# AmadeusChan/test-nccl-p2p

Hardware: AMD Instinct MI355X
Metric: pairwise P2P GB/s matrix (min/mean) + p50 latency at 1/2/4/8 MI355X (higher is better)
Workload: dtype uint8

## Files before the change

csrc/pymodule.cpp:

```cpp
#include <hip/hip_runtime.h>

#include <pybind11/pybind11.h>
#include <pybind11/stl.h>

#include <chrono>
#include <cstdlib>
#include <memory>
#include <string>
#include <thread>
#include <tuple>
#include <vector>

#include "app.hpp"
#include "bootstrap.hpp"
#include "common.hpp"
#include "kernels.hpp"
#include "provenance.hpp"
#include "report.hpp"
#include "runner.hpp"
#include "routing.hpp"
#include "schedule.hpp"
#include "transport.hpp"
#include "units.hpp"

// ... 136 lines not shown
    if (device) return ring_latency_to_json(run_device_ring_latency(*t_, *boot_, bytes, laps, warmup));
    Buffers bufs(*t_, std::max<size_t>(bytes, 16), 1);
    return ring_latency_to_json(run_ring_latency(*t_, *boot_, bytes, laps, warmup, bufs));
  }

  void set_timeout(double seconds) {
    t_->set_timeout(seconds);
    boot_->set_timeout(seconds);
  }

  bool set_chunk_cap(size_t bytes) { return t_->set_chunk_cap(bytes); }
  size_t max_chunk(int peer) const { return t_->max_chunk(peer); }
  bool refine_op_limits() { return t_->refine_op_limits(*boot_); }

  std::string link_reports() {
    const auto all = boot_->allgather_string(t_->link_report());
    std::string o = "[";
    for (size_t r = 0; r < all.size(); ++r) o += (r ? "," : "") + (all[r].empty() ? std::string("null") : all[r]);
    return o + "]";
  }

  std::string provenance(int device) { return provenance_json(*boot_, device); }

 private:
  std::unique_ptr<Bootstrap> boot_;
  std::unique_ptr<Transport> t_;
  std::string transport_kind_;
  uint64_t salt_ = 1000;
};

class PyStepDriver {
 public:
  PyStepDriver(std::shared_ptr<Session> s, const std::string& mode, const std::string& dir, size_t bytes, int msgs,
               bool verify, bool batch, bool graph, int depth, size_t recv_budget, uint64_t salt)
      : session_(std::move(s)),
        d_(std::make_unique<StepDriver>(session_->t(), session_->boot(),
                                        make_schedule(parse_mode(mode), parse_direction(dir), session_->world()),
                                        bytes, msgs, verify, salt, StepOptions{batch, graph, depth, recv_budget})) {}
  ~PyStepDriver() {
    teardown_outside_gil([this] {
      if (!session_->t().drain_quietly()) {
        (void)d_.release();
        return;
      }
      d_.reset();
    });
  }
  StepDriver& d() { return *d_; }

 private:
  std::shared_ptr<Session> session_;
  std::unique_ptr<StepDriver> d_;
};

hipStream_t as_stream(uintptr_t s) { return reinterpret_cast<hipStream_t>(s); }

struct KernelScratch {
  dev::VerifyAccum* d = nullptr;
  dev::VerifyAccum* h = nullptr;
  int device = -1;
};
KernelScratch& scratch() {
  static KernelScratch s;
  int dv = 0;
  if (hipGetDevice(&dv) != hipSuccess) P2P_FATAL("no HIP device");
  if (s.device != dv) {
    if (s.d) (void)hipFree(s.d);
    if (s.h) (void)hipHostFree(s.h);
    if (hipMalloc(&s.d, dev::verify_accum_bytes()) != hipSuccess) P2P_FATAL("hipMalloc failed");
    if (hipHostMalloc(&s.h, sizeof(dev::VerifyAccum), hipHostMallocDefault) != hipSuccess) P2P_FATAL("hipHostMalloc failed");
    s.device = dv;
// ... 228 lines not shown
      .def("device_latency", &Session::device_latency, py::arg("bytes") = 8, py::arg("iters") = 1000,
           py::arg("warmup") = 100, py::call_guard<NativeCall, py::gil_scoped_release>())
      .def("latency", &Session::latency, py::arg("bytes") = 8, py::arg("iters") = 1000, py::arg("warmup") = 100,
           py::arg("preposted") = 0, py::call_guard<NativeCall, py::gil_scoped_release>(),
           "Ping-pong matrix (collective).  preposted=B: exchanges posted B at a time behind a stream gate and "
           "released together (GPU-timeline latency; host-posted where the transport has no gate).")
      .def("fuzz", &Session::fuzz, py::arg("rounds") = 20, py::arg("seed") = 1, py::arg("max_bytes") = size_t{4} << 20,
           py::call_guard<NativeCall, py::gil_scoped_release>(),
           "Random groups of verified messages through the transport (collective); returns mismatching words.")
      .def("ring_latency", &Session::ring_latency, py::arg("bytes") = 8, py::arg("laps") = 200, py::arg("warmup") = 20,
           py::arg("device") = false, py::call_guard<NativeCall, py::gil_scoped_release>(),
           "Dependent ring token chain 0 -> 1 -> ... -> 0 (collective); JSON with per-hop and per-lap times.")
      .def("set_timeout", &Session::set_timeout, py::arg("seconds"),
           "Bounds every later wait of the session (transport sync / rendezvous, bootstrap receives).")
      .def("set_chunk_cap", &Session::set_chunk_cap, py::arg("bytes"),
           "Caps the ops messages to every peer are posted as at `bytes` (0: lifts the cap, back to the limits the "
           "transport derived per peer); False where nothing is split. Call it on every rank with the same value.")
      .def("max_chunk", &Session::max_chunk, py::arg("peer"), "Largest op a message to `peer` is posted as (0: unsplit).")
      .def("refine_op_limits", &Session::refine_op_limits, py::call_guard<NativeCall, py::gil_scoped_release>(),
           "Collective: op limits from the connections made so far (RCCL: its connection lines).")
      .def("link_reports", &Session::link_reports, py::call_guard<NativeCall, py::gil_scoped_release>(),
           "Collective: what the data plane set up towards each peer, per rank (RCCL: p2p channels from its INFO log, "
           "each peer's transport, the op limit in use); JSON list.")
      .def("provenance", &Session::provenance, py::arg("device") = -1, py::call_guard<NativeCall, py::gil_scoped_release>(),
           "Collective: runtime, RCCL library, knobs, every rank's GPU and the links between them (JSON).")
      .def("_post_unmatched_recv", &Session::post_unmatched_recv, py::arg("bytes"), py::arg("peer"),
           py::call_guard<NativeCall, py::gil_scoped_release>(),
           "Test hook: a receive no send matches, left pending; the session's teardown must still end.")
      .def("_unmatched_recv", &Session::unmatched_recv, py::arg("bytes") = size_t{1} << 20,
           py::call_guard<NativeCall, py::gil_scoped_release>(), "Test hook: a receive no send matches; returns the watchdog's error.");

  py::class_<PyStepDriver>(m, "StepDriver")
      .def(py::init<std::shared_ptr<Session>, const std::string&, const std::string&, size_t, int, bool, bool, bool, int,
                    size_t, uint64_t>(),
           py::arg("session"), py::arg("mode") = "tournament", py::arg("dir") = "bi", py::arg("bytes") = 32u << 20,
           py::arg("msgs") = 8, py::arg("verify") = false, py::arg("batch") = false, py::arg("graph") = false,
           py::arg("depth") = 1, py::arg("recv_budget") = size_t{0}, py::arg("salt") = uint64_t{0},
           py::call_guard<NativeCall, py::gil_scoped_release>())
      .def("poison", [](PyStepDriver& s) { s.d().poison(); }, py::call_guard<NativeCall, py::gil_scoped_release>(),
           "Collective: zero every receive slot (after the warmup, before the timed steps) and arm the skip faults.")
      .def("clear", [](PyStepDriver& s) { s.d().clear(); }, py::call_guard<NativeCall, py::gil_scoped_release>(),
           "Collective: zero every receive slot once every rank has drained (no fault armed).")
      .def("recapture", [](PyStepDriver& s) { s.d().recapture(); }, py::call_guard<NativeCall, py::gil_scoped_release>(),
           "Collective: record the step graphs again after the op sizes changed (no-op without graphs).")
      .def_property_readonly("recaptures", [](PyStepDriver& s) { return s.d().recaptures(); })
      .def_property_readonly("limit_changes", [](PyStepDriver& s) { return s.d().limit_changes(); })
      .def_property_readonly("graphs", [](PyStepDriver& s) { return s.d().graphs(); })
      .def("verify_steps", [](PyStepDriver& s, long first, long count) {
            StepVerifyReport r;
            {
              NativeCall in_engine;
              py::gil_scoped_release nogil;
              r = s.d().verify_steps(first, count);
            }
            py::dict d;
            d["mismatches"] = r.mismatches;
            d["verified_msgs"] = r.verified_msgs;
            d["timed_msgs"] = r.timed_msgs;
            d["slots"] = r.slots;
            return d;
          }, py::arg("first"), py::arg("count"),
           "Collective: checks every receive slot steps [first, first+count) wrote (all ranks' totals).")
      .def("flows_per_step", [](PyStepDriver& s, long k) { return s.d().flows_per_step(k); })
      .def_property_readonly("depth", [](PyStepDriver& s) { return s.d().depth(); })
      .def_property_readonly("msgs", [](PyStepDriver& s) { return s.d().msgs(); })
      .def_property_readonly("recv_bytes", [](PyStepDriver& s) { return s.d().recv_bytes(); })
      .def("connect", [](PyStepDriver& s) { s.d().connect(); }, py::call_guard<NativeCall, py::gil_scoped_release>())
      .def("step", [](PyStepDriver& s, long k) { s.d().step(k); }, py::call_guard<NativeCall, py::gil_scoped_release>())
      .def("run_steps", [](PyStepDriver& s, long first, long count) { s.d().run_steps(first, count); },
           py::call_guard<NativeCall, py::gil_scoped_release>(),
           "Enqueue steps [first, first+count); consecutive steps share their boundary timestamp.")
// ... 196 lines not shown
```

csrc/runner.hpp:

```cpp
#pragma once

#include <cstddef>
#include <cstdint>
#include <functional>
#include <string>
#include <vector>

#include "schedule.hpp"
#include "stats.hpp"
#include "transport.hpp"

namespace p2p {

class Bootstrap;

enum class Timing { Events, Wallclock };
const char* timing_name(Timing t);
Timing parse_timing(const std::string& s);

struct RunConfig {
  size_t bytes = 32u << 20;
  int iters = 128;
  int warmup = 8;
  Timing timing = Timing::Events;
// ... 102 lines not shown
struct LatencyResult {
  int a = -1, b = -1;
  size_t bytes = 0;
  Summary one_way_us;
  std::string method = "host";
};

std::vector<LatencyResult> run_latency(Transport& t, Bootstrap& boot, size_t bytes, int iters, int warmup,
                                       Buffers& bufs, int preposted = 0);

std::vector<LatencyResult> run_device_latency(Transport& t, Bootstrap& boot, size_t bytes, int iters, int warmup);

struct RingLatencyResult {
  int nranks = 0;
  size_t bytes = 0;
  int laps = 0;
  Summary hop_us;
  Summary lap_us;
  std::string method = "host";
};

RingLatencyResult run_ring_latency(Transport& t, Bootstrap& boot, size_t bytes, int laps, int warmup, Buffers& bufs);
RingLatencyResult run_device_ring_latency(Transport& t, Bootstrap& boot, size_t bytes, int laps, int warmup);

uint64_t fuzz_transport(Transport& t, Bootstrap& boot, int rounds, uint64_t seed, size_t max_bytes);

struct StepOptions {
  bool batch = false;
  bool graph = false;
  int depth = 1;
  size_t recv_budget = 0;
  int group_msgs = 0;
  int first_group_msgs = 0;
};

struct StepVerifyReport {
  uint64_t mismatches = 0;
  uint64_t verified_msgs = 0;
  uint64_t timed_msgs = 0;
  uint64_t slots = 0;
};

class StepDriver {
 public:
  StepDriver(Transport& t, Bootstrap& boot, Schedule sched, size_t bytes, int msgs, bool verify, uint64_t salt = 0,
             StepOptions opt = StepOptions());
  ~StepDriver();
  void connect();
  void step(long k);
  void run_steps(long first, long count);
  void sync();
  std::vector<double> step_ms();
  const std::vector<double>& post_ms() const { return post_ms_; }
  void reset();
  void clear();
  void poison();
  void recapture();
  int recaptures() const { return recaptures_; }
  int limit_changes() const { return limit_changes_; }
  bool graphs() const { return opt_.graph; }
  StepVerifyReport verify_steps(long first, long count);
  uint64_t verify_last();
  struct Delivery {
    const void* p = nullptr;
    int src = -1;
    int msg = 0;
  };
// ... 4 lines not shown
  int flows_per_step(long k) const;
  const Schedule& schedule() const { return sched_; }
  int phases() const { return static_cast<int>(sched_.phases.size()); }
  int depth() const { return depth_; }
  int msgs() const { return msgs_; }
  size_t recv_bytes() const { return bufs_.stride() * static_cast<size_t>(bufs_.slots()); }

  int slot_index(int rank, int gen, int phase, int msg, int i) const;
  uint64_t msg_seed(int src, int msg) const;
  size_t region_offset(int msg) const;

 private:
  Transport& t_;
  Bootstrap& boot_;
  Schedule sched_;
  size_t bytes_;
  int msgs_;
  bool verify_;
  uint64_t salt_;
  StepOptions opt_;
  std::vector<std::vector<int>> phase_base_;
  std::vector<int> gen_slots_;
  int depth_;
  Buffers bufs_;
  std::vector<std::pair<int, int>> marks_;
  std::vector<double> post_ms_;
  std::vector<int> graphs_;
  long last_step_ = -1;
  bool skip_armed_ = false;
  bool skip_some_armed_ = false;
  int recaptures_ = 0;
  int limit_changes_ = 0;
  int chain_mark_ = -1;
  int per_group_ = 0;

  void step_impl(long k, bool chain);
  void post_step_groups(const Phase& p, int pi, int gen, int per_group);
  void capture_graphs();

  void post_step_ops(const Phase& p, int pi, int gen);
  int gen_of(long k) const { return static_cast<int>((k / phases()) % depth_); }
};

}
```

csrc/step_driver.cpp:

```cpp
#include <algorithm>
#include <chrono>
#include <cstdio>
#include <cstdlib>
#include <map>
#include <string>
#include <utility>
#include <vector>

#include "bootstrap.hpp"
#include "common.hpp"
#include "prng.hpp"
#include "runner.hpp"
#include "runner_detail.hpp"

namespace p2p {

using detail::fault_applies;
using detail::flow_slots;
using detail::posts_phase;
using detail::slot_stride;

namespace {

std::vector<std::vector<int>> step_layout(const Schedule& s, int msgs) {
  P2P_CHECK(msgs >= 1, "msgs per step must be >= 1");
  std::vector<std::vector<int>> base(static_cast<size_t>(s.nranks));
  for (int r = 0; r < s.nranks; ++r) {
    int at = 0;
    for (const Phase& p : s.phases) {
      base[static_cast<size_t>(r)].push_back(at);
      at += p.recv_slots(r) * msgs;
    }
    base[static_cast<size_t>(r)].push_back(at);
  }
  return base;
}

std::vector<int> generation_sizes(const std::vector<std::vector<int>>& base) {
  std::vector<int> out;
  for (const auto& row : base) out.push_back(row.back());
  return out;
}

int agreed_depth(Transport& t, Bootstrap& boot, const StepOptions& o, size_t per_gen_bytes) {
  long d = std::max(1, o.depth);
  size_t budget = o.recv_budget;
  if (budget == 0) budget = shared_free_budget(t, boot, size_t{256} << 20, SIZE_MAX);
  if (per_gen_bytes > 0) d = std::min<long>(d, std::max<long>(1, static_cast<long>(budget / per_gen_bytes)));
  return static_cast<int>(-boot.allreduce_max(-static_cast<double>(d)));
}

}

StepDriver::StepDriver(Transport& t, Bootstrap& boot, Schedule sched, size_t bytes, int msgs, bool verify, uint64_t salt,
                       StepOptions opt)
    : t_(t), boot_(boot), sched_(std::move(sched)), bytes_(bytes), msgs_(msgs), verify_(verify), salt_(salt), opt_(opt),
      phase_base_(step_layout(sched_, msgs)), gen_slots_(generation_sizes(phase_base_)),
      depth_(agreed_depth(t, boot, opt, slot_stride(bytes) * static_cast<size_t>(gen_slots_.at(static_cast<size_t>(t.rank()))))),
      bufs_(t, bytes, std::max(1, depth_ * gen_slots_[static_cast<size_t>(t.rank())]),
            slot_stride(bytes) * static_cast<size_t>(msgs)) {
  if (opt_.graph && !t_.supports_graphs()) opt_.graph = false;
  if (const char* g = std::getenv("P2P_STEP_GROUP_MSGS"); g && opt_.group_msgs == 0) opt_.group_msgs = std::atoi(g);
  if (const char* g = std::getenv("P2P_STEP_FIRST_GROUP_MSGS"); g && opt_.first_group_msgs == 0)
    opt_.first_group_msgs = std::atoi(g);
  std::string bad = validate(sched_);
  P2P_CHECK(bad.empty(), "invalid schedule: " + bad);
  P2P_CHECK(!sched_.phases.empty(), "empty schedule");
  P2P_CHECK(sched_.nranks == t_.nranks(), "schedule and transport disagree on the number of ranks");
  for (int m = 0; m < msgs_; ++m) t_.fill(bufs_.send_at(region_offset(m)), bytes_, msg_seed(t_.rank(), m));
  if (verify_) t_.zero(bufs_.recv_base(), recv_bytes());
  t_.sync();
}

StepDriver::~StepDriver() {
  if (skip_armed_ || skip_some_armed_) t_.set_discard(false);
}

int StepDriver::slot_index(int rank, int gen, int phase, int msg, int i) const {
  const Phase& p = sched_.phases[static_cast<size_t>(phase)];
  const int r = p.recv_slots(rank);
  P2P_CHECK(i >= 0 && i < r && msg >= 0 && msg < msgs_ && gen >= 0 && gen < depth_, "bad step slot");
  return gen * gen_slots_[static_cast<size_t>(rank)] + phase_base_[static_cast<size_t>(rank)][static_cast<size_t>(phase)] +
         msg * r + i;
}

size_t StepDriver::region_offset(int msg) const { return slot_stride(bytes_) * static_cast<size_t>(msg); }

uint64_t StepDriver::msg_seed(int src, int msg) const {
  return payload_seed(src, bytes_, salt_ * 1000003ull + static_cast<uint64_t>(msg) + 1);
}

void StepDriver::connect() {
  warm_connections(t_, boot_, sched_, bufs_, std::min<size_t>(bytes_, 4096));
  for (size_t pi = 0; pi < sched_.phases.size(); ++pi)
    if (posts_phase(t_, sched_.phases[pi], t_.rank())) post_step_ops(sched_.phases[pi], static_cast<int>(pi), 0);
  t_.sync();
  boot_.barrier();
  if (verify_) t_.zero(bufs_.recv_base(), recv_bytes());
  t_.sync();
  if (t_.refine_op_limits(boot_)) ++limit_changes_;
  if (opt_.graph && graphs_.empty()) capture_graphs();
}

void StepDriver::capture_graphs() {
  for (int h : graphs_)
    if (h >= 0) t_.graph_release(h);
  graphs_.clear();
  for (int g = 0; g < depth_; ++g)
    for (size_t pi = 0; pi < sched_.phases.size(); ++pi) {
      const Phase& p = sched_.phases[pi];
      if (!p.participates(t_.rank())) {
        graphs_.push_back(-1);
        continue;
      }
      t_.capture_begin();
      post_step_ops(p, static_cast<int>(pi), g);
      graphs_.push_back(t_.capture_end());
    }
  boot_.barrier();
}

void StepDriver::recapture() {
  if (!opt_.graph) return;
  sync();
  capture_graphs();
  ++recaptures_;
}

void StepDriver::post_step_ops(const Phase& p, int pi, int gen) {
  const int me = t_.rank();
  const RankOps& ops = p.ranks[static_cast<size_t>(me)];
  const std::vector<int> rs = remote_slots(p, me);
  const bool all_flows = t_.wants_group_flows();
  std::vector<int> fslot;
  if (all_flows) fslot = flow_slots(p);
  auto one_message = [&](int m) {
    const size_t off = region_offset(m);
    if (all_flows) {
      std::vector<Transport::GroupFlow> flows(p.flows.size());
      for (size_t i = 0; i < p.flows.size(); ++i) {
        flows[i].src = p.flows[i].src;
        flows[i].dst = p.flows[i].dst;
        flows[i].slot = slot_index(p.flows[i].dst, gen, pi, m, fslot[i]);
        flows[i].src_offset = off;
      }
      t_.group_flows(bufs_.send_buf(), flows, bytes_);
    }
    for (size_t j = 0; j < ops.send_to.size(); ++j)
      t_.send_to_slot(bufs_.send_at(off), bytes_, ops.send_to[j], slot_index(ops.send_to[j], gen, pi, m, rs[j]));
    for (size_t i = 0; i < ops.recv_from.size(); ++i)
      t_.recv_from(bufs_.recv_buf(slot_index(me, gen, pi, m, static_cast<int>(i))), bytes_, ops.recv_from[i], off);
  };
  if (opt_.batch) {
    const int per = per_group_ > 0 && per_group_ < msgs_ ? per_group_ : msgs_;
    for (int m0 = 0; m0 < msgs_; m0 += per) {
      t_.group_begin();
      for (int m = m0; m < std::min(msgs_, m0 + per); ++m) one_message(m);
      t_.group_end();
    }
  } else {
    for (int m = 0; m < msgs_; ++m) {
      t_.group_begin();
      one_message(m);
      t_.group_end();
    }
  }
}

void StepDriver::post_step_groups(const Phase& p, int pi, int gen, int per_group) {
  per_group_ = per_group;
  post_step_ops(p, pi, gen);
  per_group_ = 0;
}

void StepDriver::step(long k) { step_impl(k, false); }

void StepDriver::run_steps(long first, long count) {
  for (long k = first; k < first + count; ++k) step_impl(k, k > first);
}

void StepDriver::step_impl(long k, bool chain) {
  const auto posted_from = std::chrono::steady_clock::now();
  const int pi = static_cast<int>(k % phases());
  const int g = gen_of(k);
  const Phase& p = sched_.phases[static_cast<size_t>(pi)];
  if (!chain) chain_mark_ = -1;
  if (skip_some_armed_) t_.set_discard(k % 2 == 0);
  const bool replay = opt_.graph && !skip_armed_ && !skip_some_armed_;
  const int per_group = !chain && opt_.first_group_msgs > 0 ? opt_.first_group_msgs : opt_.group_msgs;
  if (!p.participates(t_.rank())) {
    if (posts_phase(t_, p, t_.rank())) post_step_groups(p, pi, g, per_group);
    marks_.emplace_back(-1, -1);
    chain_mark_ = -1;
  } else {
    const int a = chain_mark_ >= 0 ? chain_mark_ : t_.mark();
    const size_t gi = static_cast<size_t>(g) * sched_.phases.size() + static_cast<size_t>(pi);
    if (replay && gi < graphs_.size() && graphs_[gi] >= 0)
      t_.graph_launch(graphs_[gi]);
    else
      post_step_groups(p, pi, g, per_group);
    const int b = t_.mark();
    marks_.emplace_back(a, b);
    chain_mark_ = b;
  }
  last_step_ = k;
  post_ms_.push_back(std::chrono::duration<double, std::milli>(std::chrono::steady_clock::now() - posted_from).count());
}

void StepDriver::sync() {
  t_.sync();
  std::string err = t_.async_error();
  if (!err.empty()) P2P_FATAL("transport reported an asynchronous error: " + err);
}

std::vector<double> StepDriver::step_ms() {
  std::vector<double> out;
  out.reserve(marks_.size());
  for (auto& m : marks_) out.push_back(m.first < 0 ? 0.0 : t_.elapsed_ms(m.first, m.second));
  return out;
}

void StepDriver::reset() {
  marks_.clear();
  post_ms_.clear();
  t_.clear_marks();
}

void StepDriver::clear() {
  sync();
  boot_.barrier();
  if (verify_) {
    t_.zero(bufs_.recv_base(), recv_bytes());
    t_.sync();
// ... 87 lines not shown
```

csrc/transport.hpp:

```cpp
#pragma once

#include <cstddef>
#include <cstdint>
#include <memory>
#include <string>
#include <vector>

#include "diagnose.hpp"
#include "prng.hpp"

namespace p2p {

class Bootstrap;

class Transport {
 public:
  virtual ~Transport() = default;
  virtual std::string name() const = 0;
  virtual int rank() const = 0;
  virtual int nranks() const = 0;
  virtual std::string device_desc() const { return ""; }
  virtual std::string device_key() const { return ""; }

  virtual bool mem_info(size_t* , size_t* ) { return false; }
// ... 7 lines not shown
    size_t bytes = 0;
    uint64_t seed = 0;
  };
  virtual std::vector<VerifyResult> verify_many(const std::vector<VerifyJob>& jobs) {
    std::vector<VerifyResult> out;
    out.reserve(jobs.size());
    for (const auto& j : jobs) out.push_back(verify(j.p, j.bytes, j.seed));
    return out;
  }
  virtual std::vector<DiagExtent> diagnose(const void* , size_t , uint64_t ,
                                           const std::vector<DiagCandidate>& ) {
    return {};
  }

  virtual void group_begin() = 0;
  virtual void send(const void* p, size_t bytes, int peer) = 0;
  virtual void recv(void* p, size_t bytes, int peer) = 0;
  virtual void group_end() = 0;
  virtual void recv_from(void* p, size_t bytes, int peer, size_t ) { recv(p, bytes, peer); }
  virtual void send_to_slot(const void* p, size_t bytes, int peer, int ) { send(p, bytes, peer); }
  struct GroupFlow {
    int src = -1;
    int dst = -1;
    int slot = 0;
    size_t src_offset = 0;
  };
  virtual bool wants_group_flows() const { return false; }
  virtual void group_flows(const void* , const std::vector<GroupFlow>& , size_t ) {}

  virtual int mark() = 0;
  virtual double elapsed_ms(int from, int to) = 0;
  virtual void clear_marks() = 0;
  virtual int concurrency() const { return 1; }
  virtual void sync() = 0;
  virtual bool drain_quietly() {
    try {
      sync();
      return true;
    } catch (const std::exception&) {
      return false;
    }
  }

  struct BufferSet {
    void* send = nullptr;
    size_t send_bytes = 0;
    void* recv = nullptr;
    size_t stride = 0;
    size_t slot_bytes = 0;
    int nslots = 0;
  };
  virtual void register_buffers(const BufferSet& ) {}
  virtual void unregister_buffers(void* ) {}

  virtual bool supports_graphs() const { return false; }
  virtual void capture_begin() {}
  virtual int capture_end() { return -1; }
  virtual void graph_launch(int ) {}
  virtual void graph_release(int ) {}

  virtual bool supports_device_pingpong() const { return false; }
  virtual void pingpong_setup() {}
  virtual std::vector<double> device_pingpong(int , size_t , int ) { return {}; }
  virtual std::vector<double> device_ring_token(int , int , bool , size_t ,
                                                int ) {
    return {};
// ... 68 lines not shown
```

csrc/transport_host.cpp:

```cpp
#include <arpa/inet.h>
#include <netdb.h>
#include <netinet/in.h>
#include <netinet/tcp.h>
#include <poll.h>
#include <sys/socket.h>
#include <unistd.h>

#include <algorithm>
#include <cerrno>
#include <cstdlib>
#include <cstring>
#include <deque>
#include <thread>
#include <vector>

#include "bootstrap.hpp"
#include "common.hpp"
#include "transport.hpp"

namespace p2p {

void host_fill(void* p, size_t bytes, uint64_t seed) {
  auto* b = static_cast<uint8_t*>(p);
  size_t nw = bytes / 4;
// ... 77 lines not shown
      std::string host = eps[j].host_hash == me.host_hash ? "127.0.0.1" : std::string(eps[j].host);
      fds_[j] = connect_to(host, eps[j].port);
      int32_t id = rank_;
      blocking_io(fds_[j], &id, sizeof(id), true, timeout_);
    }
    for (int got = 0; got < n_ - 1 - rank_; ++got) {
      pollfd p{lfd, POLLIN, 0};
      int rc = ::poll(&p, 1, static_cast<int>(timeout_ * 1000));
      P2P_CHECK(rc > 0, "host transport: timed out waiting for mesh connections");
      int fd = ::accept(lfd, nullptr, nullptr);
      P2P_CHECK(fd >= 0, "accept failed");
      sockopts(fd);
      int32_t id = -1;
      blocking_io(fd, &id, sizeof(id), false, timeout_);
      P2P_CHECK(id > rank_ && id < n_ && fds_[id] < 0, strfmt("bad mesh peer id %d", id));
      fds_[id] = fd;
    }
    ::close(lfd);
    boot.barrier();
  }

  ~HostTransport() override {
    release_discard_sink();
    for (int fd : fds_)
      if (fd >= 0) ::close(fd);
  }

  void set_timeout(double seconds) override { timeout_ = seconds; }
  bool gate_arm(double) override {
    const char* f = std::getenv("P2P_TEST_FAKE_GATE");
    return f && std::atoi(f) != 0;
  }
  std::string name() const override { return "host"; }
  int rank() const override { return rank_; }
  int nranks() const override { return n_; }
  std::string device_desc() const override { return "cpu:" + short_hostname(); }

  void* alloc(size_t bytes) override {
    void* p = nullptr;
    P2P_CHECK(posix_memalign(&p, 256, std::max<size_t>(bytes, 1)) == 0, "host alloc failed");
    return p;
  }
  void release(void* p) override { std::free(p); }
  void fill(void* p, size_t bytes, uint64_t seed) override { host_fill(p, bytes, seed); }
  void zero(void* p, size_t bytes) override { std::memset(p, 0, bytes); }
  VerifyResult verify(const void* p, size_t bytes, uint64_t seed) override { return host_verify(p, bytes, seed); }
  std::vector<DiagExtent> diagnose(const void* p, size_t bytes, uint64_t seed,
                                   const std::vector<DiagCandidate>& candidates) override {
    return host_diagnose_extents(p, bytes, seed, candidates);
  }

  void group_begin() override {
    P2P_CHECK(!in_group_, "nested group");
    in_group_ = true;
    ops_.clear();
  }
  void send(const void* p, size_t bytes, int peer) override {
    P2P_CHECK(peer >= 0 && peer < n_, "bad peer");
    ops_.push_back({true, peer, const_cast<char*>(static_cast<const char*>(p)), bytes});
    if (!in_group_) run_ops();
  }
  void recv(void* p, size_t bytes, int peer) override {
    P2P_CHECK(peer >= 0 && peer < n_, "bad peer");
    ops_.push_back({false, peer, static_cast<char*>(discarding() ? discard_sink(bytes) : p), bytes});
    if (!in_group_) run_ops();
  }
// ... 127 lines not shown
```

csrc/transport_ipc.cpp:

```cpp
#include <hip/hip_runtime.h>
#include <unistd.h>

#include <algorithm>
#include <array>
#include <cstdio>
#include <cstdlib>
#include <cstring>
#include <map>
#include <thread>
#include <vector>

#include "batch_verify.hpp"
#include "bootstrap.hpp"
#include "common.hpp"
#include "hip_check.hpp"
#include "kernels.hpp"
#include "provenance.hpp"
#include "routing.hpp"
#include "stream_gate.hpp"
#include "transport.hpp"
#include "units.hpp"

namespace p2p {
namespace {
// ... 32 lines not shown
    P2P_CHECK(khz > 0, "device reports no wall clock rate");
    tick_hz_ = khz * 1e3;
    if (const char* pc = std::getenv("P2P_IPC_POOL")) pool_cap_ = std::strcmp(pc, "0") ? parse_size(pc) : 0;
    if (const char* ir = std::getenv("P2P_INJECT_EXPORT_REFUSALS")) inject_refusals_ = std::atoi(ir);
    int hip_rt = 0;
    if (hipRuntimeGetVersion(&hip_rt) != hipSuccess) hip_rt = 0;
    size_fix_ = hip_rt < 70200000;
    if (const char* sf = std::getenv("P2P_IPC_SIZE_FIX")) size_fix_ = std::atoi(sf) != 0;
    if (push_) setup_sync_pages();
  }

  ~IpcTransport() override {
    (void)hipStreamSynchronize(stream_);
    if (relay_ && std::getenv("P2P_RELAY_STATS"))
      std::fprintf(stderr, "p2p_matrix: rank %d relayed %llu bytes in %llu stripes\n", rank_, relayed_bytes_,
                   relayed_stripes_);
    for (auto& r : regs_) close_registration(r);
    regs_.clear();
    release_pingpong();
    release_sync_pages();
    drain_pool();
    for (auto ex : execs_)
      if (ex) (void)hipGraphExecDestroy(ex);
    for (auto s : side_) (void)hipStreamDestroy(s);
    for (auto e : side_done_) (void)hipEventDestroy(e);
    if (fork_) (void)hipEventDestroy(fork_);
    for (auto ev : events_) (void)hipEventDestroy(ev);
    if (acc_) (void)hipFree(acc_);
    if (acc_host_) (void)hipHostFree(acc_host_);
    if (stream_) (void)hipStreamDestroy(stream_);
  }

  std::string name() const override { return "ipc"; }
  int rank() const override { return rank_; }
  int nranks() const override { return n_; }
  std::string device_desc() const override { return desc_; }
  std::string device_key() const override { return gpu_memory_key(device_); }

  bool mem_info(size_t* free_b, size_t* total_b) override {
    if (hipMemGetInfo(free_b, total_b) != hipSuccess) return false;
    *free_b += pool_bytes_;
    return true;
  }
  void* alloc(size_t bytes) override {
    constexpr size_t kGrain = size_t{2} << 20;
    size_t size = (std::max<size_t>(bytes, 1) + kGrain - 1) / kGrain * kGrain;
    constexpr size_t k4G = size_t{4} << 30;
    if (size_fix_ && size % k4G >= k4G / 2) size = (size / k4G + 1) * k4G;
    for (auto it = pool_.begin(); it != pool_.end(); ++it)
      if (it->second.size == size) {
        void* p = it->first;
        pool_bytes_ -= size;
        blocks_[p] = it->second;
        pool_.erase(it);
        return p;
      }
    Block b;
    b.size = size;
    void* p = exportable(size, &b.handle, [&](void** q) {
      hipError_t e = hipMalloc(q, size);
      if (e != hipSuccess && !pool_.empty()) {
        (void)hipGetLastError();
        drain_pool();
        e = hipMalloc(q, size);
      }
      return e;
// ... 730 lines not shown
```

csrc/transport_rccl.cpp:

```cpp
#include <hip/hip_runtime.h>
#include <rccl/rccl.h>

#include <strings.h>
#include <unistd.h>

#include <algorithm>
#include <atomic>
#include <cstdio>
#include <cstdlib>
#include <cstring>
#include <exception>
#include <fstream>
#include <sstream>
#include <thread>
#include <vector>

#include "batch_verify.hpp"
#include "bootstrap.hpp"
#include "common.hpp"
#include "hip_check.hpp"
#include "kernels.hpp"
#include "provenance.hpp"
#include "rccl_log.hpp"
#include "report.hpp"
#include "stream_gate.hpp"
#include "topology.hpp"
#include "transport.hpp"
#include "units.hpp"

namespace p2p {
namespace {

class RcclTransport final : public Transport {
 public:
  RcclTransport(Bootstrap& boot, const TransportOptions& opt)
      : rank_(boot.rank()), n_(boot.size()), timeout_(opt.timeout_s) {
    verify_impl_ = static_cast<dev::VerifyImpl>(opt.verify_impl);
    int ndev = 0;
    hipError_t e = hipGetDeviceCount(&ndev);
    if (e != hipSuccess || ndev == 0)
      P2P_FATAL(strfmt("rank %d: no HIP device visible (%s)", rank_, e == hipSuccess ? "0 devices" : hipGetErrorString(e)));
    device_ = opt.device >= 0 ? opt.device : 0;
    if (device_ >= ndev)
      P2P_FATAL(strfmt("rank %d wants GPU %d but only %d are visible: more ranks per host than GPUs", rank_, device_, ndev));
    int ncomms = opt.rccl_comms;
    if (const char* kc = std::getenv("P2P_RCCL_COMMS")) ncomms = std::atoi(kc);
    P2P_CHECK(ncomms >= 1 && ncomms <= kMaxComms, strfmt("rccl communicators per rank: 1..%d", kMaxComms));
    P2P_CHECK(ncomms == 1 || !opt.two_streams, "--two-streams (the reference layout) uses one communicator");
    HIPCHECK(hipSetDevice(device_));
    open_streams(opt, ncomms);
    stale_.assign(static_cast<size_t>(ncomms), true);
    pending_.assign(static_cast<size_t>(ncomms), false);
    unjoined_.assign(static_cast<size_t>(ncomms), false);
    send_seq_.assign(static_cast<size_t>(n_), 0);
    recv_seq_.assign(static_cast<size_t>(n_), 0);
    touched_.assign(static_cast<size_t>(n_), 0);
    HIPCHECK(hipMalloc(&acc_, dev::verify_accum_bytes()));
    HIPCHECK(hipHostMalloc(&acc_host_, sizeof(dev::VerifyAccum), hipHostMallocDefault));
    open_communicators(boot, opt, ncomms);
    describe(ncomms);
  }

  ~RcclTransport() override {
    remove_abort_hook(hook_);
    if (!drain_quietly()) {
      std::fprintf(stderr, "p2p WARN rank %d: RCCL streams still busy after the abort; leaving them to exit\n",
                   rank_);
      return;
    }
    for (auto ex : execs_)
      if (ex) (void)hipGraphExecDestroy(ex);
    for (auto g : graphs_)
      if (g) (void)hipGraphDestroy(g);
    execs_.clear();
    graphs_.clear();
    for (auto& r : reg_sets_)
      for (auto& ch : r.handles)
        if (live(ch.first)) ncclCommDeregister(ch.first, ch.second);
    reg_sets_.clear();
    try {
      release_discard_sink();
    } catch (const std::exception&) {
    }
    for (void* p : nccl_alloc_) ncclMemFree(p);
    nccl_alloc_.clear();
    for (auto& c : comms_)
// ... 118 lines not shown
      used_.resize(cstreams_.size(), false);
    }
  }
  void send(const void* p, size_t bytes, int peer) override {
    check_live("send");
    const int j = pick(&send_seq_, peer, bytes);
    touched_[static_cast<size_t>(peer)] = 1;
    sent_in_group_ = true;
    const char* c = static_cast<const char*>(p);
    do {
      size_t n = chunk_of(bytes, peer);
      issue({j, true, const_cast<char*>(c), n, peer, cstreams_[static_cast<size_t>(j)]});
      c += n;
      bytes -= n;
    } while (bytes);
  }
  void recv(void* p, size_t bytes, int peer) override {
    check_live("recv");
    const int j = pick(&recv_seq_, peer, bytes);
    touched_[static_cast<size_t>(peer)] = 1;
    const bool side = j == 0 && recv_stream_ && sent_in_group_;
    hipStream_t s = side ? recv_stream_ : cstreams_[static_cast<size_t>(j)];
    char* c = static_cast<char*>(discarding() ? discard_sink(bytes) : p);
    do {
      size_t n = chunk_of(bytes, peer);
      issue({j, false, c, n, peer, s});
      c += n;
      bytes -= n;
    } while (bytes);
    recv_on_side_ = recv_on_side_ || side;
  }
  void group_end() override {
    in_group_ = false;
    std::stable_sort(deferred_.begin(), deferred_.end(), [](const Op& a, const Op& b) { return a.comm < b.comm; });
    for (const Op& o : deferred_) post(o);
    wait_ready(ncclGroupEnd(), "ncclGroupEnd");
    deferred_.clear();
    if (recv_on_side_) {
      HIPCHECK(hipEventRecord(join_, recv_stream_));
      HIPCHECK(hipStreamWaitEvent(stream_, join_, 0));
      recv_on_side_ = false;
    }
    for (size_t j = 0; j < used_.size(); ++j)
      if (used_[j]) {
        pending_[j] = true;
        unjoined_[j] = true;
        used_[j] = false;
      }
  }

  int mark() override {
    const size_t m = static_cast<size_t>(next_event_);
    if (m == events_.size()) {
      hipEvent_t ev;
      HIPCHECK(hipEventCreateWithFlags(&ev, timing_event_flags()));
      events_.push_back(ev);
      side_ev_.emplace_back(cstreams_.size(), nullptr);
      side_rec_.emplace_back(cstreams_.size(), 0);
      side_ref_.emplace_back(cstreams_.size(), -1);
    }
    last_side_.resize(cstreams_.size(), -1);
    HIPCHECK(hipEventRecord(events_[m], stream_));
    for (size_t j = 0; j < cstreams_.size(); ++j) {
      side_rec_[m][j] = 0;
      if (j < pending_.size() && pending_[j]) {
        if (!side_ev_[m][j]) HIPCHECK(hipEventCreateWithFlags(&side_ev_[m][j], timing_event_flags()));
        HIPCHECK(hipEventRecord(side_ev_[m][j], cstreams_[j]));
        side_rec_[m][j] = 1;
        pending_[j] = false;
        last_side_[j] = static_cast<int>(m);
// ... 74 lines not shown
          P2P_FATAL(strfmt("rank %d: stream did not finish within %.0f s (peer hung or dead?); aborting", rank_, timeout_));
        }
        if (now - t0 > 20e-3) std::this_thread::sleep_for(std::chrono::microseconds(20));
      }
    }
  }

  bool drain_quietly() override {
    double deadline = now_seconds() + timeout_;
    bool aborted = false;
    for (long it = 0;; ++it) {
      bool busy = false;
      for (hipStream_t s : {stream_, recv_stream_})
        if (s && hipStreamQuery(s) == hipErrorNotReady) busy = true;
      for (auto cs : cstreams_)
        if (hipStreamQuery(cs) == hipErrorNotReady) busy = true;
      if (!busy) return true;
      const double now = now_seconds();
      const bool failed = !aborted && (it & 255) == 0 && !async_error().empty();
      if (!aborted && (failed || now > deadline || abort_requested())) {
        const bool requested = abort_requested();
        abort_all();
        if (requested) note_abort_done();
        aborted = true;
        deadline = now + 10.0;
      } else if (aborted && now > deadline) {
        return false;
      }
      std::this_thread::sleep_for(std::chrono::microseconds(100));
    }
  }

  int concurrency() const override { return static_cast<int>(comms_.size()); }
  bool set_chunk_cap(size_t bytes) override {
    cap_ = bytes;
    return true;
  }
  size_t chunk_cap() const override { return cap_; }
  std::string link_report() override { return peers_json(); }
  std::vector<std::string> peer_transports() override {
    std::vector<std::string> out;
    for (const auto& l : our_links()) out.push_back(l.transport);
    return out;
  }
  size_t max_chunk(int peer) const override { return chunk_for(peer); }

  bool gate_arm(double timeout_s) override {
    gate_.arm(stream_, timeout_s);
    return true;
  }
  void gate_release() override { gate_.release(); }
  bool gate_timed_out() override { return gate_.timed_out(); }
  void set_timeout(double seconds) override { timeout_ = seconds; }

  std::string async_error() override {
    for (auto c : comms_) {
      if (!c) return "communicator aborted";
      ncclResult_t st = ncclSuccess;
      ncclResult_t r = ncclCommGetAsyncError(c, &st);
      if (r != ncclSuccess) return ncclGetErrorString(r);
      if (st != ncclSuccess && st != ncclInProgress) return ncclGetErrorString(st);
    }
    return "";
  }

 private:
// ... 233 lines not shown
      j = static_cast<int>(key % comms_.size());
    }
    if (cstreams_[static_cast<size_t>(j)] != stream_ && !used_[static_cast<size_t>(j)]) {
      if (stale_[static_cast<size_t>(j)]) {
        if (!forked_) {
          HIPCHECK(hipEventRecord(fork_, stream_));
          forked_ = true;
        }
        HIPCHECK(hipStreamWaitEvent(cstreams_[static_cast<size_t>(j)], fork_, 0));
        stale_[static_cast<size_t>(j)] = false;
      }
      used_[static_cast<size_t>(j)] = true;
    }
    return j;
  }

  struct Op {
    int comm;
    bool send;
    char* p;
    size_t n;
    int peer;
    hipStream_t stream;
  };
  void post(const Op& o) {
    ncclComm_t c = comms_[static_cast<size_t>(o.comm)];
    if (o.send)
      nccl_ok(ncclSend(o.p, o.n, ncclUint8, o.peer, c, o.stream), "ncclSend");
    else
      nccl_ok(ncclRecv(o.p, o.n, ncclUint8, o.peer, c, o.stream), "ncclRecv");
  }
  void issue(const Op& o) {
    if (in_group_ && comms_.size() > 1)
      deferred_.push_back(o);
    else
      post(o);
  }

  void abort_all() {
    aborted_.store(true, std::memory_order_release);
    for (auto& c : comms_)
      if (c) {
        ncclCommAbort(c);
        c = nullptr;
      }
  }

  void check_live(const char* what) const {
    if (aborted_.load(std::memory_order_acquire))
      P2P_FATAL(strfmt("rank %d: %s on an aborted session: its RCCL communicators were aborted earlier (a wait that "
                       "timed out, an RCCL error or the run's deadline); open a new session",
                       rank_, what));
  }

  void nccl_ok(ncclResult_t r, const char* what) {
    if (r == ncclSuccess) return;
    if (r == ncclInProgress && nonblocking_ && !comms_.empty()) {
      wait_ready(r, what);
      return;
    }
    ncclComm_t c = comms_.empty() ? nullptr : comms_[0];
    std::string msg = strfmt("rank %d: %s failed: %s (%s)", rank_, what, ncclGetErrorString(r), c ? ncclGetLastError(c) : "") +
                      rccl_log_warnings(log_start_);
    abort_all();
    P2P_FATAL(msg);
  }

// ... 45 lines not shown
  std::vector<char> net_peer_;
  std::vector<RcclInitInfo> comm_info_;
  std::string limit_source_;
  std::vector<int> init_channels_;
  std::vector<std::string> peer_source_;
  int refinements_ = 0;
  size_t cap_ = 0;
  size_t log_start_ = 0;
  static int p2p_channel_limit(int fallback) {
    int c = fallback;
    for (const char* k : {"NCCL_MAX_P2P_NCHANNELS", "NCCL_NCHANNELS_PER_PEER"})
      if (const char* v = std::getenv(k))
        if (const int x = std::atoi(v); x > 0) c = std::min(c, x);
    return c;
  }
  size_t chunk_for(int peer) const {
    const size_t lim = peer_limit_.empty() ? 0 : peer_limit_[static_cast<size_t>(peer)];
    if (cap_ == 0) return lim;
    return lim == 0 ? cap_ : std::min(lim, cap_);
  }
  size_t chunk_of(size_t bytes, int peer) const {
    const size_t c = chunk_for(peer);
    return (c && bytes > c) ? c : bytes;
  }
  std::vector<ncclComm_t> comms_;
  std::vector<hipStream_t> cstreams_;
  std::vector<hipEvent_t> cjoin_;
  hipEvent_t fork_ = nullptr;
  bool forked_ = false;
  std::vector<bool> stale_;
  size_t split_min_ = size_t{1} << 20;
  std::vector<bool> used_;
  bool in_group_ = false;
  std::vector<Op> deferred_;
  std::vector<unsigned long long> send_seq_, recv_seq_;
  std::vector<char> touched_;
  std::vector<RcclUnparsedPeer> unparsed_;
  bool warned_unparsed_ = false;
  struct RegSet {
    void* send = nullptr;
    std::vector<std::pair<ncclComm_t, void*>> handles;
  };
  int register_ = 0;
  std::vector<RegSet> reg_sets_;
  std::vector<void*> nccl_alloc_;
  std::vector<hipEvent_t> events_;
  std::vector<std::vector<hipEvent_t>> side_ev_;
  std::vector<std::vector<char>> side_rec_;
  std::vector<std::vector<int>> side_ref_;
  std::vector<int> last_side_;
  std::vector<bool> pending_;
  std::vector<bool> unjoined_;
  std::vector<hipGraph_t> graphs_;
  std::vector<hipGraphExec_t> execs_;
  int next_event_ = 0;
  dev::VerifyAccum* acc_ = nullptr;
  dev::VerifyAccum* acc_host_ = nullptr;
  dev::BatchVerifier batch_;
  dev::Diagnoser diag_;
  dev::VerifyImpl verify_impl_ = dev::VerifyImpl::Auto;
  std::string desc_;
  int hook_ = 0;
  std::atomic<bool> aborted_{false};
  StreamGate gate_;
};

}
// ... 19 lines not shown
```

csrc/transport_shm.cpp:

```cpp
#include <fcntl.h>
#include <sys/mman.h>
#include <unistd.h>

#include <algorithm>
#include <atomic>
#include <cstdlib>
#include <cstring>
#include <deque>
#include <thread>
#include <vector>

#include "bootstrap.hpp"
#include "common.hpp"
#include "transport.hpp"
#include "units.hpp"

namespace p2p {
namespace {

constexpr size_t kLine = 64;

struct ChannelHeader {
  alignas(kLine) std::atomic<uint64_t> head;
  alignas(kLine) std::atomic<uint64_t> tail;
// ... 38 lines not shown
      P2P_CHECK(fd >= 0, strfmt("shm_open(%s): %s", seg.name, std::strerror(errno)));
      if (::ftruncate(fd, static_cast<off_t>(bytes_)) != 0) {
        ::close(fd);
        ::shm_unlink(seg.name);
        P2P_FATAL(strfmt("ftruncate of the %zu-byte shm segment: %s", bytes_, std::strerror(errno)));
      }
      map(fd);
      for (int a = 0; a < n_; ++a)
        for (int b = 0; b < n_; ++b) {
          ChannelHeader* h = header(a, b);
          new (h) ChannelHeader();
          h->head.store(0, std::memory_order_relaxed);
          h->tail.store(0, std::memory_order_relaxed);
        }
      std::atomic_thread_fence(std::memory_order_release);
    }
    boot.barrier();
    if (rank_ != 0) {
      int fd = ::shm_open(seg.name, O_RDWR, 0600);
      P2P_CHECK(fd >= 0, strfmt("shm_open(%s) on rank %d: %s", seg.name, rank_, std::strerror(errno)));
      map(fd);
    }
    boot.barrier();
    if (rank_ == 0) ::shm_unlink(seg.name);
  }

  ~ShmTransport() override {
    release_discard_sink();
    if (base_) ::munmap(base_, bytes_);
  }

  void set_timeout(double seconds) override { timeout_ = seconds; }
  std::string name() const override { return "shm"; }
  int rank() const override { return rank_; }
  int nranks() const override { return n_; }
  std::string device_desc() const override { return "cpu:" + short_hostname() + " shm"; }

  void* alloc(size_t bytes) override {
    void* p = nullptr;
    P2P_CHECK(posix_memalign(&p, 256, std::max<size_t>(bytes, 1)) == 0, "host alloc failed");
    return p;
  }
  void release(void* p) override { std::free(p); }
  void fill(void* p, size_t bytes, uint64_t seed) override { host_fill(p, bytes, seed); }
  void zero(void* p, size_t bytes) override { std::memset(p, 0, bytes); }
  VerifyResult verify(const void* p, size_t bytes, uint64_t seed) override { return host_verify(p, bytes, seed); }
  std::vector<DiagExtent> diagnose(const void* p, size_t bytes, uint64_t seed,
                                   const std::vector<DiagCandidate>& candidates) override {
    return host_diagnose_extents(p, bytes, seed, candidates);
  }

  void group_begin() override {
    P2P_CHECK(!in_group_, "nested group");
    in_group_ = true;
    ops_.clear();
  }
  void send(const void* p, size_t bytes, int peer) override {
    P2P_CHECK(peer >= 0 && peer < n_, "bad peer");
    ops_.push_back({true, peer, const_cast<char*>(static_cast<const char*>(p)), bytes});
    if (!in_group_) run_ops();
  }
  void recv(void* p, size_t bytes, int peer) override {
    P2P_CHECK(peer >= 0 && peer < n_, "bad peer");
    ops_.push_back({false, peer, static_cast<char*>(discarding() ? discard_sink(bytes) : p), bytes});
    if (!in_group_) run_ops();
  }
// ... 158 lines not shown
```

Before: 2892.

## Precompute step op lists and add ramped first-step grouping option

Step posting now uses per-phase, per-generation op lists built once, so the per-message slot index and flow computations are no longer redone on every step. Deferred RCCL ops are bucketed per communicator instead of being stable-sorted at each group end. An optional ramp splits a burst's first step into groups of L, L, 2L, 4L messages so transfers can start before the whole group is posted, but it is off by default. The prebuilt lists must be rebuilt whenever op limits or the chunk cap change, which adds state to keep consistent.

```diff
diff --git a/csrc/pymodule.cpp b/csrc/pymodule.cpp
--- a/csrc/pymodule.cpp
+++ b/csrc/pymodule.cpp
@@ -192,11 +192,13 @@
 class PyStepDriver {
  public:
   PyStepDriver(std::shared_ptr<Session> s, const std::string& mode, const std::string& dir, size_t bytes, int msgs,
-               bool verify, bool batch, bool graph, int depth, size_t recv_budget, uint64_t salt)
+               bool verify, bool batch, bool graph, int depth, size_t recv_budget, uint64_t salt, int group_msgs,
+               int first_group_msgs, int ramp_lanes)
       : session_(std::move(s)),
-        d_(std::make_unique<StepDriver>(session_->t(), session_->boot(),
-                                        make_schedule(parse_mode(mode), parse_direction(dir), session_->world()),
-                                        bytes, msgs, verify, salt, StepOptions{batch, graph, depth, recv_budget})) {}
+        d_(std::make_unique<StepDriver>(
+            session_->t(), session_->boot(), make_schedule(parse_mode(mode), parse_direction(dir), session_->world()),
+            bytes, msgs, verify, salt,
+            StepOptions{batch, graph, depth, recv_budget, group_msgs, first_group_msgs, ramp_lanes})) {}
   ~PyStepDriver() {
     teardown_outside_gil([this] {
       if (!session_->t().drain_quietly()) {
@@ -491,11 +493,15 @@
 
   py::class_<PyStepDriver>(m, "StepDriver")
       .def(py::init<std::shared_ptr<Session>, const std::string&, const std::string&, size_t, int, bool, bool, bool, int,
-                    size_t, uint64_t>(),
+                    size_t, uint64_t, int, int, int>(),
            py::arg("session"), py::arg("mode") = "tournament", py::arg("dir") = "bi", py::arg("bytes") = 32u << 20,
            py::arg("msgs") = 8, py::arg("verify") = false, py::arg("batch") = false, py::arg("graph") = false,
            py::arg("depth") = 1, py::arg("recv_budget") = size_t{0}, py::arg("salt") = uint64_t{0},
-           py::call_guard<NativeCall, py::gil_scoped_release>())
+           py::arg("group_msgs") = 0, py::arg("first_group_msgs") = 0, py::arg("ramp_lanes") = 0,
+           py::call_guard<NativeCall, py::gil_scoped_release>(),
+           "batch: messages per group of every step (group_msgs) or of a burst's first step (first_group_msgs; "
+           "-1: one group, no ramp); ramp_lanes: that first step in groups of L, L, 2L, 4L, ... messages (0: no ramp, "
+           "-1: the transport's lanes).")
       .def("poison", [](PyStepDriver& s) { s.d().poison(); }, py::call_guard<NativeCall, py::gil_scoped_release>(),
            "Collective: zero every receive slot (after the warmup, before the timed steps) and arm the skip faults.")
       .def("clear", [](PyStepDriver& s) { s.d().clear(); }, py::call_guard<NativeCall, py::gil_scoped_release>(),
diff --git a/csrc/runner.hpp b/csrc/runner.hpp
--- a/csrc/runner.hpp
+++ b/csrc/runner.hpp
@@ -158,7 +158,10 @@
   size_t recv_budget = 0;
   int group_msgs = 0;
   int first_group_msgs = 0;
-};
+  int ramp_lanes = 0;
+};
+
+std::vector<int> ramp_groups(int msgs, int lanes);
 
 struct StepVerifyReport {
   uint64_t mismatches = 0;
@@ -229,13 +232,29 @@
   int recaptures_ = 0;
   int limit_changes_ = 0;
   int chain_mark_ = -1;
-  int per_group_ = 0;
+
+  struct StepOp {
+    bool send;
+    void* p;
+    int peer;
+    int slot;
+    size_t off;
+  };
+  struct PreparedStep {
+    std::vector<StepOp> ops;
+    size_t per_msg = 0;
+    std::vector<std::vector<Transport::GroupFlow>> flows;
+  };
+  std::vector<PreparedStep> prepared_;
+  size_t prepared_cap_ = 0;
+  std::vector<int> plain_, ramp_, split_;
 
   void step_impl(long k, bool chain);
-  void post_step_groups(const Phase& p, int pi, int gen, int per_group);
   void capture_graphs();
-
-  void post_step_ops(const Phase& p, int pi, int gen);
+  void prepare_steps();
+  const std::vector<int>& equal_groups(int per);
+  const std::vector<int>& step_groups(bool chain);
+  void post_step(int pi, int gen, const std::vector<int>& groups);
   int gen_of(long k) const { return static_cast<int>((k / phases()) % depth_); }
 };
 
diff --git a/csrc/step_driver.cpp b/csrc/step_driver.cpp
--- a/csrc/step_driver.cpp
+++ b/csrc/step_driver.cpp
@@ -50,6 +50,17 @@
   return static_cast<int>(-boot.allreduce_max(-static_cast<double>(d)));
 }
 
+}
+
+std::vector<int> ramp_groups(int msgs, int lanes) {
+  P2P_CHECK(msgs >= 1, "msgs per step must be >= 1");
+  lanes = std::max(1, lanes);
+  std::vector<int> out{std::min(msgs, lanes)};
+  for (int left = msgs - out[0], next = lanes; left > 0; next *= 2) {
+    out.push_back(std::min(left, next));
+    left -= out.back();
+  }
+  return out;
 }
 
 StepDriver::StepDriver(Transport& t, Bootstrap& boot, Schedule sched, size_t bytes, int msgs, bool verify, uint64_t salt,
@@ -63,6 +74,10 @@
   if (const char* g = std::getenv("P2P_STEP_GROUP_MSGS"); g && opt_.group_msgs == 0) opt_.group_msgs = std::atoi(g);
   if (const char* g = std::getenv("P2P_STEP_FIRST_GROUP_MSGS"); g && opt_.first_group_msgs == 0)
     opt_.first_group_msgs = std::atoi(g);
+  if (const char* g = std::getenv("P2P_STEP_RAMP_LANES"); g && opt_.ramp_lanes == 0) opt_.ramp_lanes = std::atoi(g);
+  plain_ = opt_.batch ? std::vector<int>{msgs_} : std::vector<int>(static_cast<size_t>(msgs_), 1);
+  if (const int lanes = opt_.ramp_lanes < 0 ? t_.group_lanes() : opt_.ramp_lanes; lanes > 0)
+    ramp_ = ramp_groups(msgs_, lanes);
   std::string bad = validate(sched_);
   P2P_CHECK(bad.empty(), "invalid schedule: " + bad);
   P2P_CHECK(!sched_.phases.empty(), "empty schedule");
@@ -93,12 +108,16 @@
 void StepDriver::connect() {
   warm_connections(t_, boot_, sched_, bufs_, std::min<size_t>(bytes_, 4096));
   for (size_t pi = 0; pi < sched_.phases.size(); ++pi)
-    if (posts_phase(t_, sched_.phases[pi], t_.rank())) post_step_ops(sched_.phases[pi], static_cast<int>(pi), 0);
+    if (posts_phase(t_, sched_.phases[pi], t_.rank())) post_step(static_cast<int>(pi), 0, plain_);
   t_.sync();
   boot_.barrier();
   if (verify_) t_.zero(bufs_.recv_base(), recv_bytes());
   t_.sync();
-  if (t_.refine_op_limits(boot_)) ++limit_changes_;
+  if (t_.refine_op_limits(boot_)) {
+    ++limit_changes_;
+    prepared_.clear();
+  }
+  if (prepared_.empty()) prepare_steps();
   if (opt_.graph && graphs_.empty()) capture_graphs();
 }
 
@@ -114,63 +133,96 @@
         continue;
       }
       t_.capture_begin();
-      post_step_ops(p, static_cast<int>(pi), g);
+      post_step(static_cast<int>(pi), g, plain_);
       graphs_.push_back(t_.capture_end());
     }
   boot_.barrier();
 }
 
 void StepDriver::recapture() {
+  prepared_.clear();
+  prepare_steps();
   if (!opt_.graph) return;
   sync();
   capture_graphs();
   ++recaptures_;
 }
 
-void StepDriver::post_step_ops(const Phase& p, int pi, int gen) {
+void StepDriver::prepare_steps() {
   const int me = t_.rank();
-  const RankOps& ops = p.ranks[static_cast<size_t>(me)];
-  const std::vector<int> rs = remote_slots(p, me);
   const bool all_flows = t_.wants_group_flows();
-  std::vector<int> fslot;
-  if (all_flows) fslot = flow_slots(p);
-  auto one_message = [&](int m) {
-    const size_t off = region_offset(m);
-    if (all_flows) {
-      std::vector<Transport::GroupFlow> flows(p.flows.size());
-      for (size_t i = 0; i < p.flows.size(); ++i) {
-        flows[i].src = p.flows[i].src;
-        flows[i].dst = p.flows[i].dst;
-        flows[i].slot = slot_index(p.flows[i].dst, gen, pi, m, fslot[i]);
-        flows[i].src_offset = off;
+  prepared_.assign(static_cast<size_t>(depth_) * sched_.phases.size(), PreparedStep());
+  prepared_cap_ = t_.chunk_cap();
+  for (size_t pi = 0; pi < sched_.phases.size(); ++pi) {
+    const Phase& p = sched_.phases[pi];
+    if (!posts_phase(t_, p, me)) continue;
+    const RankOps& ops = p.ranks[static_cast<size_t>(me)];
+    const std::vector<int> rs = remote_slots(p, me);
+    std::vector<int> fslot;
+    if (all_flows) fslot = flow_slots(p);
+    for (int gen = 0; gen < depth_; ++gen) {
+      PreparedStep& ps = prepared_[static_cast<size_t>(gen) * sched_.phases.size() + pi];
+      ps.per_msg = ops.send_to.size() + ops.recv_from.size();
+      ps.ops.reserve(ps.per_msg * static_cast<size_t>(msgs_));
+      if (all_flows) ps.flows.resize(static_cast<size_t>(msgs_));
+      for (int m = 0; m < msgs_; ++m) {
+        const size_t off = region_offset(m);
+        if (all_flows) {
+          auto& flows = ps.flows[static_cast<size_t>(m)];
+          flows.resize(p.flows.size());
+          for (size_t i = 0; i < p.flows.size(); ++i) {
+            flows[i].src = p.flows[i].src;
+            flows[i].dst = p.flows[i].dst;
+            flows[i].slot = slot_index(p.flows[i].dst, gen, static_cast<int>(pi), m, fslot[i]);
+            flows[i].src_offset = off;
+          }
+        }
+        for (size_t j = 0; j < ops.send_to.size(); ++j)
+          ps.ops.push_back({true, bufs_.send_at(off), ops.send_to[j],
+                            slot_index(ops.send_to[j], gen, static_cast<int>(pi), m, rs[j]), 0});
+        for (size_t i = 0; i < ops.recv_from.size(); ++i)
+          ps.ops.push_back({false, bufs_.recv_buf(slot_index(me, gen, static_cast<int>(pi), m, static_cast<int>(i))),
+                            ops.recv_from[i], 0, off});
       }
-      t_.group_flows(bufs_.send_buf(), flows, bytes_);
     }
-    for (size_t j = 0; j < ops.send_to.size(); ++j)
-      t_.send_to_slot(bufs_.send_at(off), bytes_, ops.send_to[j], slot_index(ops.send_to[j], gen, pi, m, rs[j]));
-    for (size_t i = 0; i < ops.recv_from.size(); ++i)
-      t_.recv_from(bufs_.recv_buf(slot_index(me, gen, pi, m, static_cast<int>(i))), bytes_, ops.recv_from[i], off);
-  };
-  if (opt_.batch) {
-    const int per = per_group_ > 0 && per_group_ < msgs_ ? per_group_ : msgs_;
-    for (int m0 = 0; m0 < msgs_; m0 += per) {
-      t_.group_begin();
-      for (int m = m0; m < std::min(msgs_, m0 + per); ++m) one_message(m);
-      t_.group_end();
+  }
+}
+
+void StepDriver::post_step(int pi, int gen, const std::vector<int>& groups) {
+  if (prepared_.empty() || prepared_cap_ != t_.chunk_cap()) prepare_steps();
+  const PreparedStep& ps = prepared_[static_cast<size_t>(gen) * sched_.phases.size() + static_cast<size_t>(pi)];
+  const StepOp* o = ps.ops.data();
+  size_t m = 0;
+  for (int n : groups) {
+    t_.group_begin();
+    for (const size_t end = m + static_cast<size_t>(n); m < end; ++m) {
+      if (!ps.flows.empty()) t_.group_flows(bufs_.send_buf(), ps.flows[m], bytes_);
+      for (const StepOp* last = o + ps.per_msg; o < last; ++o) {
+        if (o->send)
+          t_.send_to_slot(o->p, bytes_, o->peer, o->slot);
+        else
+          t_.recv_from(o->p, bytes_, o->peer, o->off);
+      }
     }
-  } else {
-    for (int m = 0; m < msgs_; ++m) {
-      t_.group_begin();
-      one_message(m);
-      t_.group_end();
-    }
-  }
-}
-
-void StepDriver::post_step_groups(const Phase& p, int pi, int gen, int per_group) {
-  per_group_ = per_group;
-  post_step_ops(p, pi, gen);
-  per_group_ = 0;
+    t_.group_end();
+  }
+}
+
+const std::vector<int>& StepDriver::equal_groups(int per) {
+  if (per <= 0 || per >= msgs_) return plain_;
+  if (split_.empty() || split_[0] != per) {
+    split_.clear();
+    for (int m0 = 0; m0 < msgs_; m0 += per) split_.push_back(std::min(per, msgs_ - m0));
+  }
+  return split_;
+}
+
+const std::vector<int>& StepDriver::step_groups(bool chain) {
+  if (!opt_.batch) return plain_;
+  if (!chain && opt_.first_group_msgs > 0) return equal_groups(opt_.first_group_msgs);
+  if (opt_.group_msgs > 0) return equal_groups(opt_.group_msgs);
+  if (!chain && opt_.first_group_msgs == 0 && !ramp_.empty()) return ramp_;
+  return plain_;
 }
 
 void StepDriver::step(long k) { step_impl(k, false); }
@@ -187,9 +239,9 @@
   if (!chain) chain_mark_ = -1;
   if (skip_some_armed_) t_.set_discard(k % 2 == 0);
   const bool replay = opt_.graph && !skip_armed_ && !skip_some_armed_;
-  const int per_group = !chain && opt_.first_group_msgs > 0 ? opt_.first_group_msgs : opt_.group_msgs;
+  const std::vector<int>& groups = step_groups(chain);
   if (!p.participates(t_.rank())) {
-    if (posts_phase(t_, p, t_.rank())) post_step_groups(p, pi, g, per_group);
+    if (posts_phase(t_, p, t_.rank())) post_step(pi, g, groups);
     marks_.emplace_back(-1, -1);
     chain_mark_ = -1;
   } else {
@@ -198,7 +250,7 @@
     if (replay && gi < graphs_.size() && graphs_[gi] >= 0)
       t_.graph_launch(graphs_[gi]);
     else
-      post_step_groups(p, pi, g, per_group);
+      post_step(pi, g, groups);
     const int b = t_.mark();
     marks_.emplace_back(a, b);
     chain_mark_ = b;
diff --git a/csrc/transport.hpp b/csrc/transport.hpp
--- a/csrc/transport.hpp
+++ b/csrc/transport.hpp
@@ -63,6 +63,7 @@
   virtual double elapsed_ms(int from, int to) = 0;
   virtual void clear_marks() = 0;
   virtual int concurrency() const { return 1; }
+  virtual int group_lanes() const { return 1; }
   virtual void sync() = 0;
   virtual bool drain_quietly() {
     try {
diff --git a/csrc/transport_host.cpp b/csrc/transport_host.cpp
--- a/csrc/transport_host.cpp
+++ b/csrc/transport_host.cpp
@@ -133,6 +133,7 @@
     return f && std::atoi(f) != 0;
   }
   std::string name() const override { return "host"; }
+  int group_lanes() const override { return 0; }
   int rank() const override { return rank_; }
   int nranks() const override { return n_; }
   std::string device_desc() const override { return "cpu:" + short_hostname(); }
diff --git a/csrc/transport_ipc.cpp b/csrc/transport_ipc.cpp
--- a/csrc/transport_ipc.cpp
+++ b/csrc/transport_ipc.cpp
@@ -88,6 +88,7 @@
   }
 
   std::string name() const override { return "ipc"; }
+  int group_lanes() const override { return 0; }
   int rank() const override { return rank_; }
   int nranks() const override { return n_; }
   std::string device_desc() const override { return desc_; }
diff --git a/csrc/transport_rccl.cpp b/csrc/transport_rccl.cpp
--- a/csrc/transport_rccl.cpp
+++ b/csrc/transport_rccl.cpp
@@ -52,6 +52,7 @@
     stale_.assign(static_cast<size_t>(ncomms), true);
     pending_.assign(static_cast<size_t>(ncomms), false);
     unjoined_.assign(static_cast<size_t>(ncomms), false);
+    deferred_.resize(static_cast<size_t>(ncomms));
     send_seq_.assign(static_cast<size_t>(n_), 0);
     recv_seq_.assign(static_cast<size_t>(n_), 0);
     touched_.assign(static_cast<size_t>(n_), 0);
@@ -236,10 +237,10 @@
   }
   void group_end() override {
     in_group_ = false;
-    std::stable_sort(deferred_.begin(), deferred_.end(), [](const Op& a, const Op& b) { return a.comm < b.comm; });
-    for (const Op& o : deferred_) post(o);
+    for (const auto& ops : deferred_)
+      for (const Op& o : ops) post(o);
     wait_ready(ncclGroupEnd(), "ncclGroupEnd");
-    deferred_.clear();
+    for (auto& ops : deferred_) ops.clear();
     if (recv_on_side_) {
       HIPCHECK(hipEventRecord(join_, recv_stream_));
       HIPCHECK(hipStreamWaitEvent(stream_, join_, 0));
@@ -380,6 +381,7 @@
   }
 
   int concurrency() const override { return static_cast<int>(comms_.size()); }
+  int group_lanes() const override { return static_cast<int>(comms_.size()); }
   bool set_chunk_cap(size_t bytes) override {
     cap_ = bytes;
     return true;
@@ -679,7 +681,7 @@
   }
   void issue(const Op& o) {
     if (in_group_ && comms_.size() > 1)
-      deferred_.push_back(o);
+      deferred_[static_cast<size_t>(o.comm)].push_back(o);
     else
       post(o);
   }
@@ -791,7 +793,7 @@
   size_t split_min_ = size_t{1} << 20;
   std::vector<bool> used_;
   bool in_group_ = false;
-  std::vector<Op> deferred_;
+  std::vector<std::vector<Op>> deferred_;
   std::vector<unsigned long long> send_seq_, recv_seq_;
   std::vector<char> touched_;
   std::vector<RcclUnparsedPeer> unparsed_;
diff --git a/csrc/transport_shm.cpp b/csrc/transport_shm.cpp
--- a/csrc/transport_shm.cpp
+++ b/csrc/transport_shm.cpp
@@ -94,6 +94,7 @@
 
   void set_timeout(double seconds) override { timeout_ = seconds; }
   std::string name() const override { return "shm"; }
+  int group_lanes() const override { return 0; }
   int rank() const override { return rank_; }
   int nranks() const override { return n_; }
   std::string device_desc() const override { return "cpu:" + short_hostname() + " shm"; }
```

After: 2889. No clear change (-0.1%).
